# TheAustinator/keypoint-consensus-motion-correction

Measured on AMD Instinct MI355X. Metric: aligned frames/sec (whole node) at 1080p; RANSAC hypotheses scored/sec/GPU, higher is better.
Workload: dtype u16 frames; u8 descriptors: i8 MFMA exact integer distances, f64 RANSAC, f32 warp weights

## Files before the change

### include/kcmc.h

```cpp
#ifndef KCMC_H_
#define KCMC_H_

#include <stddef.h>
#include <stdint.h>

#ifdef __cplusplus
extern "C" {
#endif

#define KCMC_ABI_VERSION 2

enum {
  KCMC_OK = 0,
  KCMC_EINVAL = 1,
  KCMC_EHIP = 2,
  KCMC_ENOMEM = 3,
  KCMC_EUNSUPPORTED = 4,
  KCMC_EALIGN = 5
};

typedef struct kcmc_ctx kcmc_ctx;
typedef void* kcmc_stream_t;

int kcmc_abi_version(void);
// ... 49 lines not shown

int kcmc_consensus_vote(kcmc_ctx* ctx, const uint32_t* keep_bits_dev, int n_frames, int n_tpl,
                        long long frame_base, int64_t* out_votes_dev, kcmc_stream_t stream);
int kcmc_consensus_vote_host(const uint32_t* keep_bits_host, int n_frames, int n_tpl, long long frame_base,
                             int64_t* out_votes_host);
int kcmc_consensus_merge(const int64_t* votes_host, int world, int n_tpl, int n_kp_global, int n_min,
                         int32_t* out_consensus_host, int32_t* out_votes_host, int* out_n_consensus,
                         int32_t* out_cons_pack_host);
long long kcmc_consensus_lookup_scratch_bytes(int n_frames, int nc);
int kcmc_consensus_lookup(kcmc_ctx* ctx, const uint32_t* keep_bits_dev, int n_frames, int n_tpl,
                          const int32_t* cons_pack_dev, int nc, int32_t* out_pt_off_dev,
                          int32_t* out_pt_idx_dev, void* scratch_dev, kcmc_stream_t stream);
int kcmc_consensus_lookup_host(const uint32_t* keep_bits_host, int n_frames, int n_tpl,
                               const int32_t* cons_iter_host, int nc, int32_t* out_pt_off_host,
                               int32_t* out_pt_idx_host);

int kcmc_params_boundary(kcmc_ctx* ctx, const double* params_dev, int n_frames, int E, double* out_dev,
                         kcmc_stream_t stream);

int kcmc_hypothesis_table(int n, int trials, uint32_t seed, int min_samples, int32_t* out_host);

int kcmc_ransac_prepare(kcmc_ctx* ctx, const int32_t* n_values_host, int count, int trials, uint32_t seed);

int kcmc_ransac_rigid(kcmc_ctx* ctx, const double* src_dev, const double* dst_dev,
                      const int32_t* pt_idx_dev, const int32_t* pt_off_dev, int src_frame_stride,
                      int n_frames, int max_n, int trials, double residual_threshold,
                      double spatial_rate, int n_skip, double* out_params_dev,
                      uint8_t* out_inliers_dev, int32_t* out_n_inliers_dev,
                      int32_t* out_best_trial_dev, kcmc_stream_t stream);

int kcmc_ransac_similarity(kcmc_ctx* ctx, const double* src_dev, const double* dst_dev,
                           const int32_t* pt_idx_dev, const int32_t* pt_off_dev, int src_frame_stride,
                           int n_frames, int max_n, int trials, double residual_threshold,
                           double spatial_rate, int n_skip, double* out_params_dev,
                           uint8_t* out_inliers_dev, int32_t* out_n_inliers_dev,
                           int32_t* out_best_trial_dev, kcmc_stream_t stream);

enum { KCMC_MODEL_EUCLIDEAN = 0, KCMC_MODEL_AFFINE = 1, KCMC_MODEL_PROJECTIVE = 2, KCMC_MODEL_SIMILARITY = 3 };

int kcmc_ransac_prepare_samples(kcmc_ctx* ctx, int min_samples, const int32_t* n_values_host, int count,
                                int trials, uint32_t seed);

int kcmc_ransac_model(kcmc_ctx* ctx, int model, const double* src_dev, const double* dst_dev,
                      const int32_t* pt_idx_dev, const int32_t* pt_off_dev, int src_frame_stride,
                      int n_frames, int max_n, int trials, double residual_threshold,
                      double spatial_rate, int n_skip, double* out_params_dev,
                      uint8_t* out_inliers_dev, int32_t* out_n_inliers_dev,
                      int32_t* out_best_trial_dev, kcmc_stream_t stream);

int kcmc_warp_affine_u16(kcmc_ctx* ctx, const uint16_t* src_dev, uint16_t* dst_dev,
                         const double* M_dev, int n_frames, int H, int W, int C, int inverse_map,
                         kcmc_stream_t stream);

int kcmc_warp_perspective_u16(kcmc_ctx* ctx, const uint16_t* src_dev, uint16_t* dst_dev,
                              const double* M_dev, int n_frames, int H, int W, int C, int inverse_map,
                              kcmc_stream_t stream);

int kcmc_warp_field_u16(kcmc_ctx* ctx, const uint16_t* src_dev, uint16_t* dst_dev, const double* M_dev,
                        const int32_t* field_dev, int n_frames, int H, int W, int gy, int gx,
                        int inverse_map, kcmc_stream_t stream);

int kcmc_warp_affine_cubic_u16(kcmc_ctx* ctx, const uint16_t* src_dev, uint16_t* dst_dev,
                               const double* M_dev, int n_frames, int H, int W, int C,
                               int inverse_map, kcmc_stream_t stream);

int kcmc_histogram_u16(kcmc_ctx* ctx, const uint16_t* src_dev, unsigned long long n, int shift, int match,
                       unsigned long long* out_hist_dev, kcmc_stream_t stream);

int kcmc_lut_u16_to_u8(kcmc_ctx* ctx, const uint16_t* src_dev, unsigned long long n, const uint8_t* lut_dev,
                       uint8_t* dst_dev, kcmc_stream_t stream);

int kcmc_orb_detect(kcmc_ctx* ctx, const uint8_t* frames_dev, int n_frames, int H, int W, int threshold,
                    int n_features, double harris_k, int edge, const int8_t* pattern_dev,
                    const double* bin_cs_dev, double* out_kp_dev, uint8_t* out_des_dev,
                    int32_t* out_count_dev, kcmc_stream_t stream);

int kcmc_resize_u8(kcmc_ctx* ctx, const uint8_t* src_dev, int n_frames, int H, int W, uint8_t* dst_dev,
                   int dst_h, int dst_w, kcmc_stream_t stream);

int kcmc_orb_detect_pyramid(kcmc_ctx* ctx, const uint8_t* frames_dev, int n_frames, int H, int W, int threshold,
                            int n_features, double harris_k, int edge, const int8_t* pattern_dev,
                            const double* bin_cs_dev, int n_levels, const int32_t* level_h,
                            const int32_t* level_w, const int32_t* level_quota, double* out_kp_dev,
                            uint8_t* out_des_dev, uint8_t* out_level_dev, int32_t* out_count_dev,
                            kcmc_stream_t stream);

int kcmc_pyr_down_u8(kcmc_ctx* ctx, const uint8_t* src_dev, int n_frames, int H, int W, uint8_t* dst_dev,
                     int dst_h, int dst_w, kcmc_stream_t stream);

int kcmc_stack_sum_u16(kcmc_ctx* ctx, const uint16_t* frames_dev, int n_frames, unsigned long long n_px,
                       const uint8_t* sel_dev, long long* out_sum_dev, kcmc_stream_t stream);

int kcmc_frame_stats_u16(kcmc_ctx* ctx, const uint16_t* frames_dev, int n_frames, int H, int W,
                         const uint16_t* ref_dev, int y0, int y1, int x0, int x1, long long* out_dev,
                         kcmc_stream_t stream);

int kcmc_temporal_sums_u16(kcmc_ctx* ctx, const uint16_t* frames_dev, int n_frames, int H, int W,
                           const uint8_t* sel_dev, int y0, int y1, int x0, int x1, int neighbours,
                           long long* out_sums_dev, uint16_t* out_max_dev, kcmc_stream_t stream);

int kcmc_shift_search_u16(kcmc_ctx* ctx, const uint16_t* frames_dev, int n_frames, int H, int W,
                          const int32_t* frame_idx_dev, int n_sel, const uint16_t* ref_dev, int y0, int y1,
                          int x0, int x1, int R, long long* out_dev, kcmc_stream_t stream);

int kcmc_gradient_sums_u16(kcmc_ctx* ctx, const uint16_t* frames_dev, int n_frames, int H, int W,
                           const int32_t* frame_idx_dev, int n_sel, const uint16_t* ref_dev, int y0, int y1,
// ... 24 lines not shown
```

### keypoint-consensus-motion-correction_amd/_lib.py

```python
from __future__ import annotations

import ctypes
import os
import threading
from typing import Optional

from . import build as _build

KCMC_OK = 0
KCMC_EINVAL = 1
KCMC_EHIP = 2
KCMC_ENOMEM = 3
KCMC_EUNSUPPORTED = 4
KCMC_EALIGN = 5
ABI_VERSION = 2

EXPORTED_SYMBOLS = (
    "kcmc_abi_version",
    "kcmc_last_error",
    "kcmc_memcpy_async",
    "kcmc_create",
    "kcmc_destroy",
    "kcmc_knn2_l2u8",
    "kcmc_match_frames",
    "kcmc_match_filter",
    "kcmc_knn2_l2f32",
    "kcmc_match_frames_f32",
    "kcmc_knn2_hamming",
    "kcmc_match_frames_hamming",
    "kcmc_consensus",
    "kcmc_consensus_slice",
    "kcmc_consensus_vote",
    "kcmc_consensus_vote_host",
    "kcmc_consensus_merge",
    "kcmc_consensus_lookup_scratch_bytes",
    "kcmc_consensus_lookup",
    "kcmc_consensus_lookup_host",
    "kcmc_params_boundary",
    "kcmc_hypothesis_table",
    "kcmc_ransac_prepare",
    "kcmc_ransac_rigid",
    "kcmc_ransac_similarity",
    "kcmc_ransac_prepare_samples",
    "kcmc_ransac_model",
    "kcmc_warp_affine_u16",
    "kcmc_warp_perspective_u16",
    "kcmc_warp_field_u16",
    "kcmc_warp_affine_cubic_u16",
    "kcmc_histogram_u16",
    "kcmc_lut_u16_to_u8",
    "kcmc_orb_detect",
    "kcmc_resize_u8",
    "kcmc_orb_detect_pyramid",
    "kcmc_pyr_down_u8",
    "kcmc_stack_sum_u16",
    "kcmc_frame_stats_u16",
    "kcmc_shift_search_u16",
    "kcmc_gradient_sums_u16",
    "kcmc_tile_gradient_sums_u16",
    "kcmc_bidi_phase_sums_u16",
    "kcmc_shift_rows_u16",
    "kcmc_temporal_sums_u16",
    "kcmc_box_bandpass_u16",
    "kcmc_box_bandpass_plan",
)

KCMC_MODEL_EUCLIDEAN = 0
KCMC_MODEL_AFFINE = 1
KCMC_MODEL_PROJECTIVE = 2
KCMC_MODEL_SIMILARITY = 3
MODEL_IDS = {"euclidean": KCMC_MODEL_EUCLIDEAN, "affine": KCMC_MODEL_AFFINE, "projective": KCMC_MODEL_PROJECTIVE,
             "similarity": KCMC_MODEL_SIMILARITY}
MODEL_MIN_SAMPLES = {"euclidean": 2, "affine": 3, "projective": 4, "similarity": 2}


class KcmcLibraryError(RuntimeError):
    """libkcmc.so is missing or failed to load (no CPU fallback exists)."""


class KcmcError(RuntimeError):
    def __init__(self, code: int, msg: str):
        super().__init__(f"kcmc error {code}: {msg}")
        self.code = code
        self.msg = msg


_lock = threading.Lock()
_lib: Optional[ctypes.CDLL] = None

P = ctypes.c_void_p
I = ctypes.c_int
D = ctypes.c_double
U32 = ctypes.c_uint32
LL = ctypes.c_longlong

_SIGNATURES = {
    "kcmc_abi_version": ([], I),
    "kcmc_last_error": ([], ctypes.c_char_p),
    "kcmc_memcpy_async": ([P, P, ctypes.c_size_t, P], I),
    "kcmc_create": ([I, ctypes.POINTER(P)], I),
    "kcmc_destroy": ([P], I),
    "kcmc_knn2_l2u8": ([P, P, I, I, P, P, I, I, P, P, P], I),
    "kcmc_match_frames": ([P, P, P, I, I, P, P, P, I, I, D, D, D, P, P, P, P, P, P], I),
    "kcmc_match_filter": ([P, P, P, P, P, P, I, I, D, D, D, P, P, P, P], I),
    "kcmc_knn2_l2f32": ([P, P, I, I, P, P, I, I, P, P, P], I),
    "kcmc_match_frames_f32": ([P, P, P, I, I, P, P, P, I, I, D, D, D, P, P, P, P, P, P], I),
    "kcmc_knn2_hamming": ([P, P, I, I, P, P, I, I, P, P, P], I),
    "kcmc_match_frames_hamming": ([P, P, P, I, I, P, P, P, I, I, D, D, D, P, P, P, P, P, P], I),
    "kcmc_consensus": ([P, I, I, I, I, P, P, P, P, P], I),
    "kcmc_consensus_slice": ([P, I, I, I, I, I, I, P, P, P, P, P], I),
    "kcmc_consensus_vote": ([P, P, I, I, LL, P, P], I),
    "kcmc_consensus_vote_host": ([P, I, I, LL, P], I),
    "kcmc_consensus_merge": ([P, I, I, I, I, P, P, P, P], I),
    "kcmc_consensus_lookup_scratch_bytes": ([I, I], LL),
    "kcmc_consensus_lookup": ([P, P, I, I, P, I, P, P, P, P], I),
    "kcmc_consensus_lookup_host": ([P, I, I, P, I, P, P], I),
    "kcmc_params_boundary": ([P, P, I, I, P, P], I),
    "kcmc_hypothesis_table": ([I, I, U32, I, P], I),
    "kcmc_ransac_prepare": ([P, P, I, I, U32], I),
    "kcmc_ransac_rigid": ([P, P, P, P, P, I, I, I, I, D, D, I, P, P, P, P, P], I),
    "kcmc_ransac_similarity": ([P, P, P, P, P, I, I, I, I, D, D, I, P, P, P, P, P], I),
    "kcmc_ransac_prepare_samples": ([P, I, P, I, I, U32], I),
    "kcmc_ransac_model": ([P, I, P, P, P, P, I, I, I, I, D, D, I, P, P, P, P, P], I),
    "kcmc_warp_affine_u16": ([P, P, P, P, I, I, I, I, I, P], I),
    "kcmc_warp_perspective_u16": ([P, P, P, P, I, I, I, I, I, P], I),
    "kcmc_warp_field_u16": ([P, P, P, P, P, I, I, I, I, I, I, P], I),
    "kcmc_warp_affine_cubic_u16": ([P, P, P, P, I, I, I, I, I, P], I),
    "kcmc_histogram_u16": ([P, P, ctypes.c_ulonglong, I, I, P, P], I),
    "kcmc_lut_u16_to_u8": ([P, P, ctypes.c_ulonglong, P, P, P], I),
    "kcmc_orb_detect": ([P, P, I, I, I, I, I, D, I, P, P, P, P, P, P], I),
    "kcmc_resize_u8": ([P, P, I, I, I, P, I, I, P], I),
    "kcmc_orb_detect_pyramid": ([P, P, I, I, I, I, I, D, I, P, P, I, P, P, P, P, P, P, P, P], I),
    "kcmc_pyr_down_u8": ([P, P, I, I, I, P, I, I, P], I),
    "kcmc_stack_sum_u16": ([P, P, I, ctypes.c_ulonglong, P, P, P], I),
    "kcmc_frame_stats_u16": ([P, P, I, I, I, P, I, I, I, I, P, P], I),
    "kcmc_shift_search_u16": ([P, P, I, I, I, P, I, P, I, I, I, I, I, P, P], I),
    "kcmc_gradient_sums_u16": ([P, P, I, I, I, P, I, P, I, I, I, I, I, P, P], I),
    "kcmc_tile_gradient_sums_u16": ([P, P, I, I, I, P, I, P, P, I, P, I, P, P], I),
    "kcmc_bidi_phase_sums_u16": ([P, P, I, I, I, P, I, I, P, P], I),
    "kcmc_shift_rows_u16": ([P, P, P, I, I, I, I, I, P], I),
    "kcmc_temporal_sums_u16": ([P, P, I, I, I, P, I, I, I, I, I, P, P, P], I),
    "kcmc_box_bandpass_u16": ([P, P, P, I, I, I, I, I, P], I),
    "kcmc_box_bandpass_plan": ([I, I, I, I, I, P], I),
}


def _alt_lib() -> str:
    alt = os.environ.get("KCMC_LIB_PATH")
    if not alt:
        return ""
    if os.environ.get("KCMC_TEST_ONLY_ALT_LIB") != "1":
        raise KcmcLibraryError("KCMC_LIB_PATH is a test-only override: set KCMC_TEST_ONLY_ALT_LIB=1 as well to "
                               "load an alternative build")
    return alt


def lib_path() -> str:
    return _alt_lib() or _build.LIB_PATH


def load(auto_build: bool = True) -> ctypes.CDLL:
    global _lib
    with _lock:
        if _lib is not None:
            return _lib
        alt = _alt_lib()
        path = alt or _build.LIB_PATH
        if alt:
            import warnings

            warnings.warn(f"KCMC_LIB_PATH set: loading {path} (an A/B build; no auto-build, entry points it lacks "
                          "stay unbound and fail when called)", RuntimeWarning, stacklevel=2)
        if auto_build and os.environ.get("KCMC_NO_BUILD", "0") != "1" and not alt:
            try:
                if not _build.up_to_date():
                    _build.build()
            except Exception as e:
# ... 72 lines not shown
```

### keypoint-consensus-motion-correction_amd/csrc/warp.hip

```cpp
#include "warp_tile.h"

namespace kcmc {
namespace {

template <int TILE_H, int LDS_ELEMS, int ROW_PASSES>
struct WarpCfg {
  static constexpr int kTileH = TILE_H;
  static constexpr int kLdsElems = LDS_ELEMS;
  static constexpr int kRowPasses = ROW_PASSES;
};
using BlockCfg = WarpCfg<56, kLdsElems, kRowPasses>;
using Block64Cfg = WarpCfg<64, kLdsElems, kRowPasses>;
using ChanCfg = WarpCfg<24, 16384, 4>;

template <int C>
struct CfgFor {
  using type = std::conditional_t<C == 1, BlockCfg, ChanCfg>;
};

template <class Cfg, int C>
__device__ __forceinline__ TilePlan box_plan(long long sx0, long long sx1, long long sy0, long long sy1, int H, int W,
                                             bool small, bool stage_ok, int budget) {
  const long long ax0 = (sx0 >> 3) << 3;
  const long long pitch = ((sx1 - ax0 + 1) + 7) & ~7ll;
  const long long rows = sy1 - sy0 + 1;
  int mode = 2;
  if (small && (sx1 < 0 || sx0 > W - 1 || sy1 < 0 || sy0 > H - 1))
    mode = 1;
  else if (small && stage_ok && pitch <= kMaxPitch && rows <= 8 * Cfg::kRowPasses && pitch * rows * C <= budget)
    mode = 0;
  return TilePlan{mode, (int)ax0, (int)sy0, (int)pitch | ((int)rows << 16)};
}

template <class Cfg, int C>
__device__ __forceinline__ TilePlan source_box(const PlanTile& p, int H, int W) {
  const Box1024 b = affine_box(p.M, p.xb, p.yb, p.xl, p.yl);
  const long long sx0 = b.x0 >> 10, sx1 = (b.x1 >> 10) + 1, sy0 = b.y0 >> 10, sy1 = (b.y1 >> 10) + 1;
  const long long lim = 30000;
  const bool small = sx0 > -lim && sx1 < lim && sy0 > -lim && sy1 < lim;
  return box_plan<Cfg, C>(sx0, sx1, sy0, sy1, H, W, small, true, Cfg::kLdsElems);
}

template <class Cfg, int C>
struct BoxLoads {
  static constexpr int kPasses = C == 1 ? Cfg::kRowPasses : (Cfg::kLdsElems / 8 + kThreads - 1) / kThreads;
  uint4 chunk[kPasses];
};

template <class Cfg, int C>
__device__ __forceinline__ void box_issue(const uint16_t* __restrict__ S, const TilePlan& tp, int H, int W,
                                          BoxLoads<Cfg, C>& l) {
  if (tp.mode != 0 || (W & 7) != 0) return;
  if constexpr (C == 1) {
    stage_load(S, tp, H, W, true, l.chunk);
  } else {
    const int tid = threadIdx.x, cpr = tp.pitch() * C / 8, total = tp.rows() * cpr, rowe = W * C;
#pragma unroll
    for (int k = 0; k < BoxLoads<Cfg, C>::kPasses; ++k) {
      const int q = tid + kThreads * k;
      const int r = q / cpr, cc = q - r * cpr;
      const int gy = tp.sy0 + r;
      const int e = tp.ax0 * C + 8 * cc;
      l.chunk[k] = make_uint4(0u, 0u, 0u, 0u);
      if (q < total && (unsigned)gy < (unsigned)H && e >= 0 && e < rowe)
        l.chunk[k] = *reinterpret_cast<const uint4*>(S + (size_t)gy * rowe + e);
    }
  }
}

template <class Cfg, int C>
__device__ __forceinline__ void box_land(uint16_t* stile, const uint16_t* __restrict__ S, const TilePlan& tp, int H,
                                         int W, const BoxLoads<Cfg, C>& l) {
  if (tp.mode != 0) return;
  if constexpr (C == 1) {
    stage_commit(stile, S, tp, H, W, (W & 7) == 0, l.chunk);
  } else if ((W & 7) == 0) {
    const int tid = threadIdx.x, total = tp.rows() * (tp.pitch() * C / 8);
#pragma unroll
// ... 347 lines not shown
        }
      }
      if (hi >> 24) {
#pragma unroll
        for (int p = 0; p < 2; ++p)
#pragma unroll
          for (int k = 0; k < C; ++k)
            if (near_tie(Sx[p * C + k]))
              o[p * C + k] = blend_int(v[p][k][0], v[p][k][1], v[p][k][2], v[p][k][3], fx[p], fy[p]);
      }
    } else {
#pragma unroll
      for (int p = 0; p < 2; ++p) {
        const int X = (X0 + ad[p]) >> 5, Y = (Y0 + bd[p]) >> 5;
        if (MODE == 1) {
#pragma unroll
          for (int k = 0; k < C; ++k) o[p * C + k] = 0;
        } else {
          bilinear_px<C>(S, H, W, X, Y, o + p * C);
        }
      }
    }
    uint16_t* drow = Dst + ((size_t)y * W + x) * C;
    if (pair_store) {
      __builtin_nontemporal_store((uint32_t)o[0] | ((uint32_t)o[1] << 16), reinterpret_cast<uint32_t*>(drow));
    } else if (C >= 3 && x + 2 <= W) {
#pragma unroll
      for (int k = 0; k < C; ++k)
        __builtin_nontemporal_store((uint32_t)o[2 * k] | ((uint32_t)o[2 * k + 1] << 16),
                                    reinterpret_cast<uint32_t*>(drow) + k);
    } else {
#pragma unroll
      for (int q = 0; q < 2; ++q)
        if (x + q < W)
#pragma unroll
          for (int k = 0; k < C; ++k) drow[q * C + k] = o[q * C + k];
    }
  }
}

template <class Cfg, int C>
__device__ __forceinline__ void output_tile(const uint16_t* stile, const TilePlan& tp, const uint16_t* __restrict__ S,
                                            uint16_t* __restrict__ Dst, int H, int W, const TileId& t,
                                            const int (&ad)[2], const int (&bd)[2], int X0v, int Y0v) {
  if (tp.mode == 0)
    output_rows<Cfg, C, 0>(stile, tp, S, Dst, H, W, t, ad, bd, X0v, Y0v);
  else if (tp.mode == 1)
    output_rows<Cfg, C, 1>(stile, tp, S, Dst, H, W, t, ad, bd, X0v, Y0v);
  else
    output_rows<Cfg, C, 2>(stile, tp, S, Dst, H, W, t, ad, bd, X0v, Y0v);
}


template <int C, class Cfg>
__global__ __launch_bounds__(256) void warp_plan_kernel(const double* __restrict__ Mall, int n_frames, int H, int W,
                                                        int inverse_map, int ntx, int nty,
                                                        TilePlan* __restrict__ plan, double* __restrict__ minv,
                                                        int2* __restrict__ rowtab, int hq) {
  const long long t = blockIdx.x * (long long)blockDim.x + threadIdx.x;
  if (t >= (long long)ntx * nty * n_frames) return;
  const PlanTile p = plan_tile<Cfg::kTileH>(t, Mall, inverse_map, H, W, ntx, nty, minv);
  TilePlan b = source_box<Cfg, C>(p, H, W);
  if ((W & 7) == 0 && (C > 1 || 2ll * H * W < (1ll << 31)) && b.mode == 0 && b.pitch() <= kFastPitch &&
      b.rows() <= Fast<Cfg, C>::kRows)
    b.mode = 3;
  if (map_has_nan(p.M, 6)) b.mode = 1;
  plan[t] = b;
  for (int j = p.xb / kTileW; j < Cfg::kTileH && p.yb + j < H; j += ntx) {
    const int y = p.yb + j;
    rowtab[((size_t)p.f * 4 + (y & 3)) * hq + (y >> 2)] =
        make_int2(cv_round((p.M[1] * y + p.M[2]) * 1024) + 16, cv_round((p.M[4] * y + p.M[5]) * 1024) + 16);
  }
}

template <int C, class Cfg = BlockCfg>
__global__ __launch_bounds__(kThreads) __attribute__((target("no-unaligned-access-mode"))) void warp_affine_u16_kernel(
    const uint16_t* __restrict__ src, uint16_t* __restrict__ dst, const TilePlan* __restrict__ plan,
    const double* __restrict__ minv, const int2* __restrict__ rowtab, int hq, int H, int W) {
  __shared__ __attribute__((aligned(16))) uint16_t stile[Cfg::kLdsElems];
  const TileId t = tile_decode<Cfg::kTileH>();
  const int tid = threadIdx.x;
  const uint16_t* S = src + (size_t)t.f * H * W * C;
  uint16_t* Dst = dst + (size_t)t.f * H * W * C;
  const double* M = minv + 6 * (size_t)t.f;

  const TilePlan tp = plan[t.tile];
  KCMC_LDS_SENTINEL(stile, Cfg::kLdsElems, tid);
  int ad[2], bd[2];
  if (tp.mode == 3) {
    using F = Fast<Cfg, C>;
    typename F::Loads loads;
    F::issue(S, tp, H, W, tid, loads);
    lane_columns(M, t.xb, t.lane, W, ad, bd);
    const uint32_t nb = F::land(stile, tp, tid, loads);
    uint32_t* flags = reinterpret_cast<uint32_t*>(stile) + F::kFlagWord;
    if (t.lane == 0) flags[t.wave] = nb;
    __syncthreads();
    const uint4 fl = *reinterpret_cast<const uint4*>(flags);
    const uint32_t bright = fl.x + fl.y + fl.z + fl.w;
    const int2* rt = rowtab + ((size_t)t.f * 4 + t.wave) * hq + (t.yb >> 2);
    const int ox = tp.ax0 * 1024, oy = tp.sy0 * 1024;
    const bool interior = t.yb + Cfg::kTileH <= H && t.xb + kTileW <= W;
#define KCMC_FAST_ROWS(blend, inside) \
  fast_rows<Cfg, C, blend, inside>(stile, rt, ox, oy, Dst, H, W, t.xb, t.yb, t.wave, t.lane, ad, bd)
    if (bright == 0) {
      if (interior)
        KCMC_FAST_ROWS(kDark, true);
      else
        KCMC_FAST_ROWS(kDark, false);
    } else if ((int)bright * kBrightShare <= tp.rows() * (tp.pitch() >> 3)) {
      if (interior)
        KCMC_FAST_ROWS(kMixed, true);
      else
        KCMC_FAST_ROWS(kMixed, false);
    } else {
      KCMC_FAST_ROWS(kBright, false);
    }
#undef KCMC_FAST_ROWS
    return;
  }
  BoxLoads<Cfg, C> loads;
  box_issue<Cfg, C>(S, tp, H, W, loads);
  int X0v, Y0v;
  lane_columns(M, t.xb, t.lane, W, ad, bd);
  row_origins<Cfg::kTileH>(M, t, tp, X0v, Y0v);
  box_land<Cfg, C>(stile, S, tp, H, W, loads);
  __syncthreads();
  output_tile<Cfg, C>(stile, tp, S, Dst, H, W, t, ad, bd, X0v, Y0v);
}


__device__ __forceinline__ void invert_perspective(const double* S, double* M) {
  double d = S[0] * (S[4] * S[8] - S[5] * S[7]) - S[1] * (S[3] * S[8] - S[5] * S[6]) +
             S[2] * (S[3] * S[7] - S[4] * S[6]);
  if (d == 0.0) {
    for (int k = 0; k < 9; ++k) M[k] = 0.0;
    return;
  }
  d = 1. / d;
  M[0] = (S[4] * S[8] - S[5] * S[7]) * d;
  M[1] = (S[2] * S[7] - S[1] * S[8]) * d;
  M[2] = (S[1] * S[5] - S[2] * S[4]) * d;
  M[3] = (S[5] * S[6] - S[3] * S[8]) * d;
  M[4] = (S[0] * S[8] - S[2] * S[6]) * d;
  M[5] = (S[2] * S[3] - S[0] * S[5]) * d;
  M[6] = (S[3] * S[7] - S[4] * S[6]) * d;
  M[7] = (S[1] * S[6] - S[0] * S[7]) * d;
  M[8] = (S[0] * S[4] - S[1] * S[3]) * d;
}

template <class Cfg>
struct PerspTab {
  static constexpr int kEntries = Cfg::kTileH * 2;
  static constexpr int kElems = kEntries * 3 * 4;
  static constexpr int kFlagWord = Cfg::kLdsElems / 2 - 4;
  static constexpr int kBoxElems = Cfg::kLdsElems - 8 - kElems;
  static_assert((kBoxElems * 2) % 8 == 0, "table alignment");
};

template <class Cfg, int C>
__device__ __forceinline__ TilePlan persp_box(const double* M, int xb, int yb, int H, int W) {
  const int xl = min(xb + kTileW, W) - 1, yl = min(yb + Cfg::kTileH, H) - 1;
  const int cx[4] = {xb, xl, xb, xl}, cy[4] = {yb, yb, yl, yl};
  double mnx = INFINITY, mxx = -INFINITY, mny = INFINITY, mxy = -INFINITY;
  bool pos = true, neg = true, wrange = true;
#pragma unroll
  for (int k = 0; k < 4; ++k) {
    const double w = M[6] * cx[k] + M[7] * cy[k] + M[8];
    pos = pos && w > 0.0;
    neg = neg && w < 0.0;
    wrange = wrange && fabs(w) >= 0x1p-56 && fabs(w) <= 0x1p56;
    const double sx = (M[0] * cx[k] + M[1] * cy[k] + M[2]) / w;
    const double sy = (M[3] * cx[k] + M[4] * cy[k] + M[5]) / w;
    mnx = fmin(mnx, sx);
    mxx = fmax(mxx, sx);
    mny = fmin(mny, sy);
    mxy = fmax(mxy, sy);
// ... 201 lines not shown
  KCMC_LDS_SENTINEL(stile, Cfg::kLdsElems, tid);
  BoxLoads<Cfg, C> loads;
  box_issue<Cfg, C>(S, tp, H, W, loads);
  double M[9];
#pragma unroll
  for (int k = 0; k < 9; ++k) M[k] = minv[9 * (size_t)t.f + k];
  double* ptab = reinterpret_cast<double*>(stile + PerspTab<Cfg>::kBoxElems);
  const bool tab = bw0 == 64 && tp.mode != 1;
  if (tab) {
    for (int e = tid; e < PerspTab<Cfg>::kEntries; e += kThreads) {
      const double dy = (double)(t.yb + (e >> 1)), dxo = (double)(t.xb + 64 * (e & 1));
      ptab[3 * e] = M[0] * dxo + M[1] * dy + M[2];
      ptab[3 * e + 1] = M[3] * dxo + M[4] * dy + M[5];
      ptab[3 * e + 2] = M[6] * dxo + M[7] * dy + M[8];
    }
  }
  const bool count = C == 1 && (W & 7) == 0;
  uint32_t* flags = reinterpret_cast<uint32_t*>(stile) + PerspTab<Cfg>::kFlagWord;
  if (tp.mode == 0) {
    box_land<Cfg, C>(stile, S, tp, H, W, loads);
    if (count) {
      uint32_t nb = 0;
#pragma unroll
      for (int k = 0; k < BoxLoads<Cfg, C>::kPasses; ++k) nb += bright_chunks(loads.chunk[k]);
      if (t.lane == 0) flags[t.wave] = nb;
    }
  }
  __syncthreads();
  if (tp.mode == 1)
    persp_rows<Cfg, C, 1, false>(stile, tp, S, Dst, M, H, W, t, bw0, ptab);
  else if (tab) {
    if (tp.mode == 0) {
      const uint4 fl = *reinterpret_cast<const uint4*>(flags);
      if (count && fl.x + fl.y + fl.z + fl.w == 0)
        persp_rows<Cfg, C, 0, true, true>(stile, tp, S, Dst, M, H, W, t, bw0, ptab);
      else
        persp_rows<Cfg, C, 0, true>(stile, tp, S, Dst, M, H, W, t, bw0, ptab);
    } else
      persp_rows<Cfg, C, 2, true>(stile, tp, S, Dst, M, H, W, t, bw0, ptab);
  } else if (tp.mode == 0) {
    persp_rows<Cfg, C, 0, false>(stile, tp, S, Dst, M, H, W, t, bw0, ptab);
  } else {
    persp_rows<Cfg, C, 2, false>(stile, tp, S, Dst, M, H, W, t, bw0, ptab);
  }
}

inline int rowtab_hq(int H) { return ceil_div(H, 4) + 16; }

inline int persp_bw0(int H, int W) {
  const int bh0 = H < 16 ? H : 16;
  return 1024 / bh0 < W ? 1024 / bh0 : W;
}

template <class Cfg>
struct LinearWs {
  int ntx, nty, hq;
  long long tiles;
  size_t tab_at, plan_at, bytes;
  LinearWs(bool perspective, int n_frames, int H, int W) {
    ntx = ceil_div(W, kTileW), nty = ceil_div(H, Cfg::kTileH);
    tiles = (long long)ntx * nty * n_frames;
    hq = perspective ? 0 : rowtab_hq(H);
    tab_at = (size_t)n_frames * (perspective ? 9 : 6) * sizeof(double);
    plan_at = tab_at + (size_t)n_frames * 4 * hq * sizeof(int2);
    bytes = plan_at + (size_t)tiles * sizeof(TilePlan);
  }
  double* minv(void* ws) const { return static_cast<double*>(ws); }
  int2* rowtab(void* ws) const { return reinterpret_cast<int2*>(static_cast<char*>(ws) + tab_at); }
  TilePlan* plan(void* ws) const { return reinterpret_cast<TilePlan*>(static_cast<char*>(ws) + plan_at); }
};

template <class Cfg>
size_t warp_workspace_bytes(int n_frames, int H, int W) {
  return LinearWs<Cfg>(false, n_frames, H, W).bytes;
}

template <bool PERSP, int C, class Cfg>
void launch_linear(const uint16_t* src, uint16_t* dst, const double* M, int n_frames, int H, int W, int inverse_map,
                   void* ws, hipStream_t s) {
  const LinearWs<Cfg> w(PERSP, n_frames, H, W);
  const dim3 plan_grid((unsigned)((w.tiles + 255) / 256)), tile_grid(w.ntx, w.nty, n_frames);
  if constexpr (PERSP) {
    hipLaunchKernelGGL((persp_plan_kernel<C, Cfg>), plan_grid, dim3(256), 0, s, M, n_frames, H, W, inverse_map, w.ntx,
                       w.nty, w.plan(ws), w.minv(ws));
    hipLaunchKernelGGL((warp_perspective_u16_kernel<C, Cfg>), tile_grid, dim3(kThreads), 0, s, src, dst, w.plan(ws),
                       w.minv(ws), H, W, persp_bw0(H, W));
  } else {
    hipLaunchKernelGGL((warp_plan_kernel<C, Cfg>), plan_grid, dim3(256), 0, s, M, n_frames, H, W, inverse_map, w.ntx,
                       w.nty, w.plan(ws), w.minv(ws), w.rowtab(ws), w.hq);
    hipLaunchKernelGGL((warp_affine_u16_kernel<C, Cfg>), tile_grid, dim3(kThreads), 0, s, src, dst, w.plan(ws),
                       w.minv(ws), w.rowtab(ws), w.hq, H, W);
  }
}

template <int C, class Cfg = typename CfgFor<C>::type>
void launch_warp(const uint16_t* src, uint16_t* dst, const double* M, int n_frames, int H, int W, int inverse_map,
                 void* ws, hipStream_t s) {
  launch_linear<false, C, Cfg>(src, dst, M, n_frames, H, W, inverse_map, ws, s);
}

template <bool PERSP, int C, class Cfg>
struct LinearCfg {
  static constexpr bool kPersp = PERSP;
  static constexpr int kC = C;
  using cfg = Cfg;
};

template <bool PERSP, typename F>
int with_linear_cfg(int C, int H, F f) {
  if constexpr (!PERSP)
    if (C == 1 && use_tile64(H)) return f(LinearCfg<PERSP, 1, Block64Cfg>());
  if (C == 1) return f(LinearCfg<PERSP, 1, BlockCfg>());
  return C == 3 ? f(LinearCfg<PERSP, 3, ChanCfg>()) : f(LinearCfg<PERSP, 4, ChanCfg>());
}

template <typename F>
int with_linear_cfg(bool perspective, int C, int H, F f) {
  return perspective ? with_linear_cfg<true>(C, H, f) : with_linear_cfg<false>(C, H, f);
}

int run_linear_warp(const char* name, const char* kernel_name, bool perspective, kcmc_ctx* ctx, const uint16_t* src,
                    uint16_t* dst, const double* M, int n_frames, int H, int W, int C, int inverse_map,
                    kcmc_stream_t stream) {
  const std::string w(name);
  if (!ctx) return fail(KCMC_EINVAL, w + ": ctx is NULL");
  if (n_frames < 0 || H < 0 || W < 0) return fail(KCMC_EINVAL, w + ": negative size");
  if (H > 32767 || W > 32767) return fail(KCMC_EUNSUPPORTED, w + ": H, W must be < 32768");
  if (n_frames > 65535) return fail(KCMC_EUNSUPPORTED, w + ": at most 65535 frames per call");
  if (C != 1 && C != 3 && C != 4) return fail(KCMC_EUNSUPPORTED, w + ": C must be 1, 3 or 4");
  if ((long long)ceil_div(W, kTileW) * ceil_div(H, ChanCfg::kTileH) * n_frames >= (1ll << 31))
    return fail(KCMC_EUNSUPPORTED, w + ": too many tiles in one call");
  if (n_frames == 0 || H == 0 || W == 0) return KCMC_OK;
  if (!src || !dst || !M) return fail(KCMC_EINVAL, w + ": NULL pointer");
  if (src == dst) return fail(KCMC_EINVAL, w + ": in-place warp is not supported");
  hipStream_t s = (hipStream_t)stream;
  return with_linear_cfg(perspective, C, H, [&](auto k) -> int {
    using K = decltype(k);
    void* ws = nullptr;
    const size_t wsb = LinearWs<typename K::cfg>(K::kPersp, n_frames, H, W).bytes;
    KCMC_TRY(workspace_alloc(ctx, &ws, wsb, s));
    launch_linear<K::kPersp, K::kC, typename K::cfg>(src, dst, M, n_frames, H, W, inverse_map, ws, s);
    const int rc = launch_check(kernel_name);
    KCMC_TRY(workspace_free(ctx, ws, s, wsb));
    return rc;
  });
}

}
}

using namespace kcmc;

extern "C" int kcmc_warp_perspective_u16(kcmc_ctx* ctx, const uint16_t* src, uint16_t* dst, const double* M,
                                         int n_frames, int H, int W, int C, int inverse_map, kcmc_stream_t stream) {
  return run_linear_warp("kcmc_warp_perspective_u16", "warp_perspective_u16_kernel", true, ctx, src, dst, M, n_frames,
                         H, W, C, inverse_map, stream);
}

extern "C" int kcmc_warp_affine_u16(kcmc_ctx* ctx, const uint16_t* src, uint16_t* dst, const double* M,
                                    int n_frames, int H, int W, int C, int inverse_map, kcmc_stream_t stream) {
  return run_linear_warp("kcmc_warp_affine_u16", "warp_affine_u16_kernel", false, ctx, src, dst, M, n_frames, H, W, C,
                         inverse_map, stream);
}
```

Measured before the change: 658,400.

## Replace per-tile warp plans with per-frame row/column/band tables

The default affine warp now runs a per-frame table kernel instead of the per-tile plan kernel. That kernel precomputes fixed-point row offsets, column offsets and per-tile-row/column bounding bands. The warp kernel rebuilds each tile's source box from two band entries and loads its lane column offsets from the table, instead of recomputing them from the double-precision matrix. This removes per-tile double math and per-lane column arithmetic, at the cost of a table kernel with one block per frame, extra workspace and 32-bit box arithmetic. The old tile-plan path stays available through a new _planned entry point.

Result: no change. 661,700 (median of 6 runs) (+0.5%).

```diff
diff --git a/include/kcmc.h b/include/kcmc.h
--- a/include/kcmc.h
+++ b/include/kcmc.h
@@ -125,6 +125,10 @@
                          const double* M_dev, int n_frames, int H, int W, int C, int inverse_map,
                          kcmc_stream_t stream);
 
+int kcmc_warp_affine_u16_planned(kcmc_ctx* ctx, const uint16_t* src_dev, uint16_t* dst_dev,
+                                 const double* M_dev, int n_frames, int H, int W, int C, int inverse_map,
+                                 kcmc_stream_t stream);
+
 int kcmc_warp_perspective_u16(kcmc_ctx* ctx, const uint16_t* src_dev, uint16_t* dst_dev,
                               const double* M_dev, int n_frames, int H, int W, int C, int inverse_map,
                               kcmc_stream_t stream);
diff --git a/keypoint-consensus-motion-correction_amd/_lib.py b/keypoint-consensus-motion-correction_amd/_lib.py
--- a/keypoint-consensus-motion-correction_amd/_lib.py
+++ b/keypoint-consensus-motion-correction_amd/_lib.py
@@ -44,6 +44,7 @@
     "kcmc_ransac_prepare_samples",
     "kcmc_ransac_model",
     "kcmc_warp_affine_u16",
+    "kcmc_warp_affine_u16_planned",
     "kcmc_warp_perspective_u16",
     "kcmc_warp_field_u16",
     "kcmc_warp_affine_cubic_u16",
@@ -123,6 +124,7 @@
     "kcmc_ransac_prepare_samples": ([P, I, P, I, I, U32], I),
     "kcmc_ransac_model": ([P, I, P, P, P, P, I, I, I, I, D, D, I, P, P, P, P, P], I),
     "kcmc_warp_affine_u16": ([P, P, P, P, I, I, I, I, I, P], I),
+    "kcmc_warp_affine_u16_planned": ([P, P, P, P, I, I, I, I, I, P], I),
     "kcmc_warp_perspective_u16": ([P, P, P, P, I, I, I, I, I, P], I),
     "kcmc_warp_field_u16": ([P, P, P, P, P, I, I, I, I, I, I, P], I),
     "kcmc_warp_affine_cubic_u16": ([P, P, P, P, I, I, I, I, I, P], I),
diff --git a/keypoint-consensus-motion-correction_amd/csrc/warp.hip b/keypoint-consensus-motion-correction_amd/csrc/warp.hip
--- a/keypoint-consensus-motion-correction_amd/csrc/warp.hip
+++ b/keypoint-consensus-motion-correction_amd/csrc/warp.hip
@@ -18,12 +18,12 @@
   using type = std::conditional_t<C == 1, BlockCfg, ChanCfg>;
 };
 
-template <class Cfg, int C>
-__device__ __forceinline__ TilePlan box_plan(long long sx0, long long sx1, long long sy0, long long sy1, int H, int W,
-                                             bool small, bool stage_ok, int budget) {
-  const long long ax0 = (sx0 >> 3) << 3;
-  const long long pitch = ((sx1 - ax0 + 1) + 7) & ~7ll;
-  const long long rows = sy1 - sy0 + 1;
+template <class Cfg, int C, typename I>
+__device__ __forceinline__ TilePlan box_plan(I sx0, I sx1, I sy0, I sy1, int H, int W, bool small, bool stage_ok,
+                                             int budget) {
+  const I ax0 = (sx0 >> 3) << 3;
+  const I pitch = ((sx1 - ax0 + 1) + 7) & ~(I)7;
+  const I rows = sy1 - sy0 + 1;
   int mode = 2;
   if (small && (sx1 < 0 || sx0 > W - 1 || sy1 < 0 || sy0 > H - 1))
     mode = 1;
@@ -477,6 +477,74 @@
 }
 
 
+template <class Cfg, int C>
+__device__ __forceinline__ TilePlan finish_plan(TilePlan b, int H, int W, bool has_nan) {
+  if ((W & 7) == 0 && (C > 1 || (uint32_t)H * (uint32_t)W < (1u << 30)) && b.mode == 0 && b.pitch() <= kFastPitch &&
+      b.rows() <= Fast<Cfg, C>::kRows)
+    b.mode = 3;
+  if (has_nan) b.mode = 1;
+  return b;
+}
+
+struct FrameTables {
+  const int2* rowtab;
+  const int2* coltab;
+  const int4* band;
+  const int* nan;
+  int hq, wpad;
+};
+
+template <class Cfg, int C>
+__device__ __forceinline__ TilePlan table_plan(const FrameTables& ft, const TileId& t, int H, int W) {
+  const int ntx = gridDim.x, nty = gridDim.y;
+  const int4* bf = ft.band + t.f * (ntx + nty);
+  const int4 rb = bf[t.yb / Cfg::kTileH], cb = bf[nty + t.xb / kTileW];
+  const int has_nan = ft.nan[t.f];
+  const int sx0 = (int)(((long long)rb.x + cb.x) >> 10), sx1 = (int)(((long long)rb.y + cb.y) >> 10) + 1;
+  const int sy0 = (int)(((long long)rb.z + cb.z) >> 10), sy1 = (int)(((long long)rb.w + cb.w) >> 10) + 1;
+  const int lim = 30000;
+  const bool small = min(sx0, sy0) > -lim && max(sx1, sy1) < lim;
+  return finish_plan<Cfg, C>(box_plan<Cfg, C>(sx0, sx1, sy0, sy1, H, W, small, true, Cfg::kLdsElems), H, W,
+                             has_nan != 0);
+}
+
+constexpr int kTableThreads = 256;
+__global__ __launch_bounds__(kTableThreads) void warp_frame_tables_kernel(
+    const double* __restrict__ Mall, int H, int W, int inverse_map, int tile_h, double* __restrict__ minv,
+    int2* __restrict__ rowtab, int hq, int2* __restrict__ coltab, int wpad, int4* __restrict__ band,
+    int* __restrict__ nan) {
+  const int f = blockIdx.x, tid = threadIdx.x;
+  double M[6];
+  load_map(Mall, f, inverse_map, M);
+  if (tid == 0) {
+    for (int k = 0; k < 6; ++k) minv[6 * (size_t)f + k] = M[k];
+    nan[f] = map_has_nan(M, 6) ? 1 : 0;
+  }
+  for (int y = tid; y < H; y += kTableThreads)
+    rowtab[((size_t)f * 4 + (y & 3)) * hq + (y >> 2)] =
+        make_int2(cv_round((M[1] * y + M[2]) * 1024) + 16, cv_round((M[4] * y + M[5]) * 1024) + 16);
+  for (int x0 = tid; x0 < wpad; x0 += kTableThreads) {
+    const int x = min(x0, W - 1);
+    coltab[(size_t)f * wpad + x0] = make_int2(cv_round(M[0] * x * 1024), cv_round(M[3] * x * 1024));
+  }
+  const int ntx = wpad / kTileW, nty = (H + tile_h - 1) / tile_h;
+  for (int i = tid; i < nty + ntx; i += kTableThreads) {
+    int4 e;
+    if (i < nty) {
+      const int yb = i * tile_h, yl = min(yb + tile_h, H) - 1;
+      const int x0 = cv_round((M[1] * yb + M[2]) * 1024) + 16, x1 = cv_round((M[1] * yl + M[2]) * 1024) + 16;
+      const int y0 = cv_round((M[4] * yb + M[5]) * 1024) + 16, y1 = cv_round((M[4] * yl + M[5]) * 1024) + 16;
+      e = make_int4(min(x0, x1), max(x0, x1), min(y0, y1), max(y0, y1));
+    } else {
+      const int xb = (i - nty) * kTileW, xl = min(xb + kTileW, W) - 1;
+      const int a0 = cv_round(M[0] * xb * 1024), a1 = cv_round(M[0] * xl * 1024);
+      const int b0 = cv_round(M[3] * xb * 1024), b1 = cv_round(M[3] * xl * 1024);
+      e = make_int4(min(a0, a1), max(a0, a1), min(b0, b1), max(b0, b1));
+    }
+    band[(size_t)f * (nty + ntx) + i] = e;
+  }
+}
+
 template <int C, class Cfg>
 __global__ __launch_bounds__(256) void warp_plan_kernel(const double* __restrict__ Mall, int n_frames, int H, int W,
                                                         int inverse_map, int ntx, int nty,
@@ -485,12 +553,7 @@
   const long long t = blockIdx.x * (long long)blockDim.x + threadIdx.x;
   if (t >= (long long)ntx * nty * n_frames) return;
   const PlanTile p = plan_tile<Cfg::kTileH>(t, Mall, inverse_map, H, W, ntx, nty, minv);
-  TilePlan b = source_box<Cfg, C>(p, H, W);
-  if ((W & 7) == 0 && (C > 1 || 2ll * H * W < (1ll << 31)) && b.mode == 0 && b.pitch() <= kFastPitch &&
-      b.rows() <= Fast<Cfg, C>::kRows)
-    b.mode = 3;
-  if (map_has_nan(p.M, 6)) b.mode = 1;
-  plan[t] = b;
+  plan[t] = finish_plan<Cfg, C>(source_box<Cfg, C>(p, H, W), H, W, map_has_nan(p.M, 6));
   for (int j = p.xb / kTileW; j < Cfg::kTileH && p.yb + j < H; j += ntx) {
     const int y = p.yb + j;
     rowtab[((size_t)p.f * 4 + (y & 3)) * hq + (y >> 2)] =
@@ -498,25 +561,44 @@
   }
 }
 
-template <int C, class Cfg = BlockCfg>
+__device__ __forceinline__ int4 lane_columns_load(const FrameTables& ft, const TileId& t) {
+  return *reinterpret_cast<const int4*>(ft.coltab + t.f * ft.wpad + t.xb + 2 * t.lane);
+}
+__device__ __forceinline__ void lane_columns_land(const int4& c, int (&ad)[2], int (&bd)[2]) {
+  ad[0] = c.x, bd[0] = c.y, ad[1] = c.z, bd[1] = c.w;
+}
+
+template <int C, class Cfg = BlockCfg, bool TABLES = true>
 __global__ __launch_bounds__(kThreads) __attribute__((target("no-unaligned-access-mode"))) void warp_affine_u16_kernel(
     const uint16_t* __restrict__ src, uint16_t* __restrict__ dst, const TilePlan* __restrict__ plan,
-    const double* __restrict__ minv, const int2* __restrict__ rowtab, int hq, int H, int W) {
+    const double* __restrict__ minv, const int2* __restrict__ rowtab, int hq, const int2* __restrict__ coltab, int wpad,
+    const int4* __restrict__ band, const int* __restrict__ nan, int H, int W) {
   __shared__ __attribute__((aligned(16))) uint16_t stile[Cfg::kLdsElems];
   const TileId t = tile_decode<Cfg::kTileH>();
   const int tid = threadIdx.x;
   const uint16_t* S = src + (size_t)t.f * H * W * C;
   uint16_t* Dst = dst + (size_t)t.f * H * W * C;
   const double* M = minv + 6 * (size_t)t.f;
-
-  const TilePlan tp = plan[t.tile];
+  const FrameTables ft{rowtab, coltab, band, nan, hq, wpad};
+
+  TilePlan tp;
+  int4 cols = make_int4(0, 0, 0, 0);
+  if constexpr (TABLES) {
+    cols = lane_columns_load(ft, t);
+    tp = table_plan<Cfg, C>(ft, t, H, W);
+  } else {
+    tp = plan[t.tile];
+  }
   KCMC_LDS_SENTINEL(stile, Cfg::kLdsElems, tid);
   int ad[2], bd[2];
   if (tp.mode == 3) {
     using F = Fast<Cfg, C>;
     typename F::Loads loads;
     F::issue(S, tp, H, W, tid, loads);
-    lane_columns(M, t.xb, t.lane, W, ad, bd);
+    if constexpr (TABLES)
+      lane_columns_land(cols, ad, bd);
+    else
+      lane_columns(M, t.xb, t.lane, W, ad, bd);
     const uint32_t nb = F::land(stile, tp, tid, loads);
     uint32_t* flags = reinterpret_cast<uint32_t*>(stile) + F::kFlagWord;
     if (t.lane == 0) flags[t.wave] = nb;
@@ -547,7 +629,10 @@
   BoxLoads<Cfg, C> loads;
   box_issue<Cfg, C>(S, tp, H, W, loads);
   int X0v, Y0v;
-  lane_columns(M, t.xb, t.lane, W, ad, bd);
+  if constexpr (TABLES)
+    lane_columns_land(cols, ad, bd);
+  else
+    lane_columns(M, t.xb, t.lane, W, ad, bd);
   row_origins<Cfg::kTileH>(M, t, tp, X0v, Y0v);
   box_land<Cfg, C>(stile, S, tp, H, W, loads);
   __syncthreads();
@@ -855,74 +940,92 @@
   return 1024 / bh0 < W ? 1024 / bh0 : W;
 }
 
+inline int coltab_wpad(int W) { return ceil_div(W, kTileW) * kTileW; }
+
+enum PlanSource { kFromTables, kFromTilePlans, kFromPerspPlans };
+
 template <class Cfg>
 struct LinearWs {
-  int ntx, nty, hq;
+  int ntx, nty, hq, wpad;
   long long tiles;
-  size_t tab_at, plan_at, bytes;
-  LinearWs(bool perspective, int n_frames, int H, int W) {
+  size_t tab_at, col_at, band_at, tail_at, bytes;
+  LinearWs(PlanSource ps, int n_frames, int H, int W) {
     ntx = ceil_div(W, kTileW), nty = ceil_div(H, Cfg::kTileH);
     tiles = (long long)ntx * nty * n_frames;
-    hq = perspective ? 0 : rowtab_hq(H);
-    tab_at = (size_t)n_frames * (perspective ? 9 : 6) * sizeof(double);
-    plan_at = tab_at + (size_t)n_frames * 4 * hq * sizeof(int2);
-    bytes = plan_at + (size_t)tiles * sizeof(TilePlan);
+    hq = ps == kFromPerspPlans ? 0 : rowtab_hq(H);
+    wpad = ps == kFromTables ? coltab_wpad(W) : 0;
+    tab_at = (size_t)n_frames * (ps == kFromPerspPlans ? 9 : 6) * sizeof(double);
+    col_at = tab_at + (size_t)n_frames * 4 * hq * sizeof(int2);
+    band_at = col_at + (size_t)n_frames * wpad * sizeof(int2);
+    tail_at = band_at + (ps == kFromTables ? (size_t)n_frames * (nty + ntx) * sizeof(int4) : 0);
+    bytes = tail_at + (ps == kFromTables ? (size_t)n_frames * sizeof(int) : (size_t)tiles * sizeof(TilePlan));
   }
   double* minv(void* ws) const { return static_cast<double*>(ws); }
   int2* rowtab(void* ws) const { return reinterpret_cast<int2*>(static_cast<char*>(ws) + tab_at); }
-  TilePlan* plan(void* ws) const { return reinterpret_cast<TilePlan*>(static_cast<char*>(ws) + plan_at); }
+  int2* coltab(void* ws) const { return reinterpret_cast<int2*>(static_cast<char*>(ws) + col_at); }
+  int4* band(void* ws) const { return reinterpret_cast<int4*>(static_cast<char*>(ws) + band_at); }
+  int* nan(void* ws) const { return reinterpret_cast<int*>(static_cast<char*>(ws) + tail_at); }
+  TilePlan* plan(void* ws) const { return reinterpret_cast<TilePlan*>(static_cast<char*>(ws) + tail_at); }
 };
 
 template <class Cfg>
 size_t warp_workspace_bytes(int n_frames, int H, int W) {
-  return LinearWs<Cfg>(false, n_frames, H, W).bytes;
-}
-
-template <bool PERSP, int C, class Cfg>
+  return LinearWs<Cfg>(kFromTables, n_frames, H, W).bytes;
+}
+
+template <PlanSource PS, int C, class Cfg>
 void launch_linear(const uint16_t* src, uint16_t* dst, const double* M, int n_frames, int H, int W, int inverse_map,
                    void* ws, hipStream_t s) {
-  const LinearWs<Cfg> w(PERSP, n_frames, H, W);
+  const LinearWs<Cfg> w(PS, n_frames, H, W);
   const dim3 plan_grid((unsigned)((w.tiles + 255) / 256)), tile_grid(w.ntx, w.nty, n_frames);
-  if constexpr (PERSP) {
+  if constexpr (PS == kFromPerspPlans) {
     hipLaunchKernelGGL((persp_plan_kernel<C, Cfg>), plan_grid, dim3(256), 0, s, M, n_frames, H, W, inverse_map, w.ntx,
                        w.nty, w.plan(ws), w.minv(ws));
     hipLaunchKernelGGL((warp_perspective_u16_kernel<C, Cfg>), tile_grid, dim3(kThreads), 0, s, src, dst, w.plan(ws),
                        w.minv(ws), H, W, persp_bw0(H, W));
-  } else {
+  } else if constexpr (PS == kFromTilePlans) {
     hipLaunchKernelGGL((warp_plan_kernel<C, Cfg>), plan_grid, dim3(256), 0, s, M, n_frames, H, W, inverse_map, w.ntx,
                        w.nty, w.plan(ws), w.minv(ws), w.rowtab(ws), w.hq);
-    hipLaunchKernelGGL((warp_affine_u16_kernel<C, Cfg>), tile_grid, dim3(kThreads), 0, s, src, dst, w.plan(ws),
-                       w.minv(ws), w.rowtab(ws), w.hq, H, W);
+    hipLaunchKernelGGL((warp_affine_u16_kernel<C, Cfg, false>), tile_grid, dim3(kThreads), 0, s, src, dst, w.plan(ws),
+                       w.minv(ws), w.rowtab(ws), w.hq, (const int2*)nullptr, 0, (const int4*)nullptr,
+                       (const int*)nullptr, H, W);
+  } else {
+    hipLaunchKernelGGL(warp_frame_tables_kernel, dim3(n_frames), dim3(kTableThreads), 0, s, M, H, W, inverse_map,
+                       Cfg::kTileH, w.minv(ws), w.rowtab(ws), w.hq, w.coltab(ws), w.wpad, w.band(ws), w.nan(ws));
+    hipLaunchKernelGGL((warp_affine_u16_kernel<C, Cfg, true>), tile_grid, dim3(kThreads), 0, s, src, dst,
+                       (const TilePlan*)nullptr, w.minv(ws), w.rowtab(ws), w.hq, w.coltab(ws), w.wpad, w.band(ws),
+                       w.nan(ws), H, W);
   }
 }
 
 template <int C, class Cfg = typename CfgFor<C>::type>
 void launch_warp(const uint16_t* src, uint16_t* dst, const double* M, int n_frames, int H, int W, int inverse_map,
                  void* ws, hipStream_t s) {
-  launch_linear<false, C, Cfg>(src, dst, M, n_frames, H, W, inverse_map, ws, s);
-}
-
-template <bool PERSP, int C, class Cfg>
+  launch_linear<kFromTables, C, Cfg>(src, dst, M, n_frames, H, W, inverse_map, ws, s);
+}
+
+template <PlanSource PS, int C, class Cfg>
 struct LinearCfg {
-  static constexpr bool kPersp = PERSP;
+  static constexpr PlanSource kSource = PS;
   static constexpr int kC = C;
   using cfg = Cfg;
 };
 
-template <bool PERSP, typename F>
+template <PlanSource PS, typename F>
 int with_linear_cfg(int C, int H, F f) {
-  if constexpr (!PERSP)
-    if (C == 1 && use_tile64(H)) return f(LinearCfg<PERSP, 1, Block64Cfg>());
-  if (C == 1) return f(LinearCfg<PERSP, 1, BlockCfg>());
-  return C == 3 ? f(LinearCfg<PERSP, 3, ChanCfg>()) : f(LinearCfg<PERSP, 4, ChanCfg>());
+  if constexpr (PS != kFromPerspPlans)
+    if (C == 1 && use_tile64(H)) return f(LinearCfg<PS, 1, Block64Cfg>());
+  if (C == 1) return f(LinearCfg<PS, 1, BlockCfg>());
+  return C == 3 ? f(LinearCfg<PS, 3, ChanCfg>()) : f(LinearCfg<PS, 4, ChanCfg>());
 }
 
 template <typename F>
-int with_linear_cfg(bool perspective, int C, int H, F f) {
-  return perspective ? with_linear_cfg<true>(C, H, f) : with_linear_cfg<false>(C, H, f);
-}
-
-int run_linear_warp(const char* name, const char* kernel_name, bool perspective, kcmc_ctx* ctx, const uint16_t* src,
+int with_linear_cfg(PlanSource ps, int C, int H, F f) {
+  if (ps == kFromPerspPlans) return with_linear_cfg<kFromPerspPlans>(C, H, f);
+  return ps == kFromTables ? with_linear_cfg<kFromTables>(C, H, f) : with_linear_cfg<kFromTilePlans>(C, H, f);
+}
+
+int run_linear_warp(const char* name, const char* kernel_name, PlanSource ps, kcmc_ctx* ctx, const uint16_t* src,
                     uint16_t* dst, const double* M, int n_frames, int H, int W, int C, int inverse_map,
                     kcmc_stream_t stream) {
   const std::string w(name);
@@ -937,12 +1040,12 @@
   if (!src || !dst || !M) return fail(KCMC_EINVAL, w + ": NULL pointer");
   if (src == dst) return fail(KCMC_EINVAL, w + ": in-place warp is not supported");
   hipStream_t s = (hipStream_t)stream;
-  return with_linear_cfg(perspective, C, H, [&](auto k) -> int {
+  return with_linear_cfg(ps, C, H, [&](auto k) -> int {
     using K = decltype(k);
     void* ws = nullptr;
-    const size_t wsb = LinearWs<typename K::cfg>(K::kPersp, n_frames, H, W).bytes;
+    const size_t wsb = LinearWs<typename K::cfg>(K::kSource, n_frames, H, W).bytes;
     KCMC_TRY(workspace_alloc(ctx, &ws, wsb, s));
-    launch_linear<K::kPersp, K::kC, typename K::cfg>(src, dst, M, n_frames, H, W, inverse_map, ws, s);
+    launch_linear<K::kSource, K::kC, typename K::cfg>(src, dst, M, n_frames, H, W, inverse_map, ws, s);
     const int rc = launch_check(kernel_name);
     KCMC_TRY(workspace_free(ctx, ws, s, wsb));
     return rc;
@@ -956,12 +1059,18 @@
 
 extern "C" int kcmc_warp_perspective_u16(kcmc_ctx* ctx, const uint16_t* src, uint16_t* dst, const double* M,
                                          int n_frames, int H, int W, int C, int inverse_map, kcmc_stream_t stream) {
-  return run_linear_warp("kcmc_warp_perspective_u16", "warp_perspective_u16_kernel", true, ctx, src, dst, M, n_frames,
-                         H, W, C, inverse_map, stream);
+  return run_linear_warp("kcmc_warp_perspective_u16", "warp_perspective_u16_kernel", kFromPerspPlans, ctx, src, dst, M,
+                         n_frames, H, W, C, inverse_map, stream);
 }
 
 extern "C" int kcmc_warp_affine_u16(kcmc_ctx* ctx, const uint16_t* src, uint16_t* dst, const double* M,
                                     int n_frames, int H, int W, int C, int inverse_map, kcmc_stream_t stream) {
-  return run_linear_warp("kcmc_warp_affine_u16", "warp_affine_u16_kernel", false, ctx, src, dst, M, n_frames, H, W, C,
-                         inverse_map, stream);
-}
+  return run_linear_warp("kcmc_warp_affine_u16", "warp_affine_u16_kernel", kFromTables, ctx, src, dst, M, n_frames, H, W,
+                         C, inverse_map, stream);
+}
+
+extern "C" int kcmc_warp_affine_u16_planned(kcmc_ctx* ctx, const uint16_t* src, uint16_t* dst, const double* M,
+                                            int n_frames, int H, int W, int C, int inverse_map, kcmc_stream_t stream) {
+  return run_linear_warp("kcmc_warp_affine_u16_planned", "warp_affine_u16_kernel", kFromTilePlans, ctx, src, dst, M,
+                         n_frames, H, W, C, inverse_map, stream);
+}
```
